# XUANTIE-RV/csi-nn2

Measured on AMD Instinct MI355X. Metric: mobilenetv1_int8_images_per_sec, higher is better.
Workload: dtype i8; 1 GPU; mobilenetv1 int8 NHWC batch 1/GPU, 28 conv layers in 15 launches, hipGraph replay via csinn_*; ops_per_image=1137480704, algorithmic_bytes_per_image=8323144, algorithmic_bytes_per_image_survey=14444616, parallelism=replicas x1

## Files before the change

### csi-nn2_amd/csrc/stemdw_fused.hip

```cpp
#include <stdio.h>
#include <stdlib.h>

#include "dw_patch.h"

namespace shl {

struct StemDwArgs {
    ConvArgs st;
    ConvArgs dw;
    int32_t bh, bw;
    int32_t tiles_x, tiles_y;
    int32_t rw, npx;
    uint32_t rw_magic, bw_magic;
};

template <int EPQ, int EPD>
__global__ __launch_bounds__(256) void stemdw_fused_kernel(StemDwArgs f)
{
    extern __shared__ __attribute__((aligned(16))) char smem[];
    const ConvArgs &q = f.st;
    const ConvArgs &d = f.dw;
    asm volatile("" ::"s"(q.in), "s"(q.w), "s"(q.acc_init), "s"(q.mult), "s"(q.bias), "s"(q.H), "s"(q.W), "s"(q.Ho), "s"(q.Wo), "s"(q.sh),
                 "s"(q.sw), "s"(q.pt), "s"(q.pl), "s"(q.dh), "s"(q.dw), "s"(q.in_zp));
    asm volatile("" ::"s"(f.bh), "s"(f.bw), "s"(f.tiles_y), "s"(f.rw), "s"(f.npx), "s"(f.rw_magic), "s"(f.bw_magic), "s"(d.N), "s"(d.sh),
                 "s"(d.sw), "s"(d.pt), "s"(d.pl), "s"(d.w), "s"(d.acc_init), "s"(d.mult), "s"(d.bias), "s"(d.out));
    asm volatile("" ::"s"(q.out_zp), "s"(q.out_zp_f), "s"(q.clamp_lo), "s"(q.clamp_hi), "s"(d.out_zp), "s"(d.out_zp_f), "s"(d.clamp_lo),
                 "s"(d.clamp_hi), "s"(d.in_zp), "s"(d.Ho), "s"(d.Wo), "s"(d.H), "s"(d.W), "s"(d.C));
    const int tid = threadIdx.x;
    int32_t *w_lds = reinterpret_cast<int32_t *>(smem);
    int32_t *t_tab = w_lds + 7 * 32;
    uint32_t *patch = reinterpret_cast<uint32_t *>(t_tab + 96);
    if (tid < 224) w_lds[tid] = static_cast<const int32_t *>(q.w)[tid];
    if (tid < 96) {
        const int which = tid >> 5, i = tid & 31;
        t_tab[tid] = which == 0 ? q.acc_init[i] : which == 1 ? __float_as_int(q.mult[i]) : __float_as_int(q.bias[i]);
    }
    const int tx = blockIdx.x;
    int ty = blockIdx.y, n = 0;
    if (d.N > 1) {
        n = ty / f.tiles_y;
        ty -= n * f.tiles_y;
    }
    const int oy0 = ty * f.bh, ox0 = tx * f.bw;
    const int ry0 = oy0 * d.sh - d.pt, rx0 = ox0 * d.sw - d.pl;
    const DwThreadConsts dwk = dw_load_consts(d, 0, tid);

    const int8_t *img = static_cast<const int8_t *>(q.in) + (int64_t)n * q.H * q.W * 3;
    const int ntasks = 2 * f.npx;
    const int ppitch = dw_patch_pitch(f.npx);
    const uint32_t zpad = dw_patch_pad(d);
    for (int base = 0; base < ntasks; base += 256) {
        const bool valid = base + tid < ntasks;
        const int task = valid ? base + tid : ntasks - 1;
        const int j = task >> 1, cb = (task & 1) * 16;
        const int pr = (int)(((uint32_t)j * f.rw_magic) >> 20);
        const int pc = j - pr * f.rw;
        const int sy = ry0 + pr, sx = rx0 + pc;
        const bool inside = (unsigned)sy < (unsigned)q.Ho && (unsigned)sx < (unsigned)q.Wo;
        const int y0 = sy * q.sh - q.pt, x0 = sx * q.sw - q.pl;
        int qv[28];
#pragma unroll
        for (int ky = 0; ky < 3; ++ky)
#pragma unroll
            for (int kx = 0; kx < 3; ++kx) {
                const int y = y0 + ky * q.dh, x = x0 + kx * q.dw;
                const bool ok = inside && (unsigned)y < (unsigned)q.H && (unsigned)x < (unsigned)q.W;
                const int8_t *px = img + ((int64_t)y * q.W + x) * 3;
#pragma unroll
                for (int c = 0; c < 3; ++c) qv[(ky * 3 + kx) * 3 + c] = ok ? (int)px[c] : q.in_zp;
            }
        qv[27] = 0;
        uint32_t q4[7];
#pragma unroll
        for (int g = 0; g < 7; ++g)
            q4[g] = (uint32_t)(qv[4 * g] & 0xFF) | ((uint32_t)(qv[4 * g + 1] & 0xFF) << 8) |
                    ((uint32_t)(qv[4 * g + 2] & 0xFF) << 16) | ((uint32_t)(qv[4 * g + 3] & 0xFF) << 24);
        if (base == 0) __syncthreads();
        int acc[16];
#pragma unroll
        for (int e = 0; e < 16; ++e) acc[e] = 0;
#pragma unroll
        for (int g = 0; g < 7; ++g)
#pragma unroll
            for (int v = 0; v < 4; ++v) {
                const int4 w = *reinterpret_cast<const int4 *>(&w_lds[g * 32 + cb + 4 * v]);
                acc[4 * v + 0] = __builtin_amdgcn_sdot4((int)q4[g], w.x, acc[4 * v + 0], false);
                acc[4 * v + 1] = __builtin_amdgcn_sdot4((int)q4[g], w.y, acc[4 * v + 1], false);
                acc[4 * v + 2] = __builtin_amdgcn_sdot4((int)q4[g], w.z, acc[4 * v + 2], false);
                acc[4 * v + 3] = __builtin_amdgcn_sdot4((int)q4[g], w.w, acc[4 * v + 3], false);
            }
#pragma unroll
        for (int v = 0; v < 4; ++v) {
            const int c = cb + 4 * v;
            const int4 ai = *reinterpret_cast<const int4 *>(t_tab + c);
            const float4 mu = *reinterpret_cast<const float4 *>(t_tab + 32 + c);
            const float4 bi = *reinterpret_cast<const float4 *>(t_tab + 64 + c);
            const uint32_t pk = requant4_i8_sel<EPQ>(acc[4 * v] + ai.x, acc[4 * v + 1] + ai.y, acc[4 * v + 2] + ai.z,
                                               acc[4 * v + 3] + ai.w, mu, bi, q);
            if (valid) patch[dw_patch_slot(j, c >> 2, ppitch)] = inside ? pk : zpad;
        }
    }
    __syncthreads();

    DwPatchGeom g;
    g.bh = f.bh, g.bw = f.bw, g.rw = f.rw, g.bw_magic = f.bw_magic, g.pitch = ppitch;
    g.oy0 = oy0, g.ox0 = ox0, g.ry0 = ry0, g.rx0 = rx0, g.n = n, g.ch0 = 0;
    depthwise_from_patch<EPD>(d, patch, g, dwk, tid, 256);
}

static bool stemdw_geometry(const ConvArgs &q, const ConvArgs &d, StemDwArgs &f)
{
    if (q.Kh != 3 || q.Kw != 3 || q.C != 3 || q.Co != 32) return false;
    if (d.Kh != 3 || d.Kw != 3 || d.dh != 1 || d.dw != 1 || d.C != 32 || d.Co != 32) return false;
    if (d.H != q.Ho || d.W != q.Wo || d.N != q.N || d.sh < 1 || d.sh > 2 || d.sw < 1 || d.sw > 2) return false;
    if (d.pt < 0 || d.pl < 0 || d.pt > 2 || d.pl > 2) return false;
    if ((int64_t)d.Ho * d.Wo * d.C >= ((int64_t)1 << 31)) return false;
    f.bh = d.Ho < 2 ? d.Ho : 2;
    f.bw = d.Wo < 28 ? d.Wo : 28;
    if (const char *e = getenv("SHL_MI355X_STEMDW_TILE")) {
        int h = 0, w = 0;
        if (sscanf(e, "%dx%d", &h, &w) == 2 && h > 0 && w > 0) f.bh = h < d.Ho ? h : d.Ho, f.bw = w < d.Wo ? w : d.Wo;
    }
    f.tiles_y = (d.Ho + f.bh - 1) / f.bh;
    f.tiles_x = (d.Wo + f.bw - 1) / f.bw;
    f.rw = (f.bw - 1) * d.sw + 3;
    f.npx = ((f.bh - 1) * d.sh + 3) * f.rw;
    f.rw_magic = ((1u << 20) + f.rw - 1) / f.rw;
    f.bw_magic = ((1u << 20) + f.bw - 1) / f.bw;
    if (f.npx >= 2048 || f.tiles_x > 65535 || (int64_t)f.tiles_y * d.N > 65535) return false;
    return (int64_t)f.tiles_x * f.tiles_y * d.N <= 2048;
}

bool stemdw_fusable(const ConvArgs &q, const ConvArgs &d)
{
    StemDwArgs f;
    return stemdw_geometry(q, d, f);
}

int launch_stemdw_fused(const ConvArgs &q, const ConvArgs &d, hipStream_t s)
{
    StemDwArgs f;
    f.st = q;
    f.dw = d;
    if (!stemdw_geometry(q, d, f)) {
        set_error("stemdw_fused: the pair does not qualify");
        return SHL_MI355X_ENOTSUP;
    }
    const dim3 grid((unsigned)f.tiles_x, (unsigned)(f.tiles_y * d.N));
    const size_t lds = (size_t)(7 * 32 + 96) * 4 + dw_patch_bytes(f.npx);
    const int epq = (q.act != SHL_MI355X_ACT_NONE && !q.act_clamp) ? -1 : (q.div_exact ? 3 : 0);
    const int epd = (d.act != SHL_MI355X_ACT_NONE && !d.act_clamp) ? -1 : (d.div_exact ? 3 : 0);
    if (epq == 3 && epd == 3) hipLaunchKernelGGL((stemdw_fused_kernel<3, 3>), grid, dim3(256), lds, s, f);
    else if (epq == 0 && epd == 0) hipLaunchKernelGGL((stemdw_fused_kernel<0, 0>), grid, dim3(256), lds, s, f);
    else hipLaunchKernelGGL((stemdw_fused_kernel<-1, -1>), grid, dim3(256), lds, s, f);
    SHL_HIP(hipGetLastError());
    return SHL_MI355X_OK;
}

}
```

Baseline: 17580 img/s.

## Compute stem conv with MFMA i8 from an LDS-staged input patch in stem+dw fusion

The stem 3x3x3->32 conv inside the fused stem+depthwise kernel switches from per-thread sdot4 loops (27 global byte loads per task) to a path that first stages the raw input patch into LDS with buffer byte loads. It then builds im2col fragments with alignbyte and runs one mfma_i32_32x32x32_i8 per 32-pixel tile per wave. Weights and requant constants now sit in registers instead of LDS. This is meant to cut redundant global input loads and ALU dot-product work, at the cost of more register pressure, extra LDS for the input patch, and a new launch variant chosen by patch size. It is on by default and can be disabled with an environment variable.

```diff
diff --git a/csi-nn2_amd/csrc/stemdw_fused.hip b/csi-nn2_amd/csrc/stemdw_fused.hip
--- a/csi-nn2_amd/csrc/stemdw_fused.hip
+++ b/csi-nn2_amd/csrc/stemdw_fused.hip
@@ -12,9 +12,13 @@
     int32_t tiles_x, tiles_y;
     int32_t rw, npx;
     uint32_t rw_magic, bw_magic;
+    int32_t mfma;
+    int32_t ir, ipd;
+    uint32_t ipd_magic;
+    int32_t mt;
 };
 
-template <int EPQ, int EPD>
+template <int EPQ, int EPD, bool MFMA, int NI = 0>
 __global__ __launch_bounds__(256) void stemdw_fused_kernel(StemDwArgs f)
 {
     extern __shared__ __attribute__((aligned(16))) char smem[];
@@ -26,15 +30,8 @@
                  "s"(d.sw), "s"(d.pt), "s"(d.pl), "s"(d.w), "s"(d.acc_init), "s"(d.mult), "s"(d.bias), "s"(d.out));
     asm volatile("" ::"s"(q.out_zp), "s"(q.out_zp_f), "s"(q.clamp_lo), "s"(q.clamp_hi), "s"(d.out_zp), "s"(d.out_zp_f), "s"(d.clamp_lo),
                  "s"(d.clamp_hi), "s"(d.in_zp), "s"(d.Ho), "s"(d.Wo), "s"(d.H), "s"(d.W), "s"(d.C));
+    if constexpr (MFMA) asm volatile("" ::"s"(f.ir), "s"(f.ipd), "s"(f.ipd_magic), "s"(f.mt));
     const int tid = threadIdx.x;
-    int32_t *w_lds = reinterpret_cast<int32_t *>(smem);
-    int32_t *t_tab = w_lds + 7 * 32;
-    uint32_t *patch = reinterpret_cast<uint32_t *>(t_tab + 96);
-    if (tid < 224) w_lds[tid] = static_cast<const int32_t *>(q.w)[tid];
-    if (tid < 96) {
-        const int which = tid >> 5, i = tid & 31;
-        t_tab[tid] = which == 0 ? q.acc_init[i] : which == 1 ? __float_as_int(q.mult[i]) : __float_as_int(q.bias[i]);
-    }
     const int tx = blockIdx.x;
     int ty = blockIdx.y, n = 0;
     if (d.N > 1) {
@@ -43,61 +40,158 @@
     }
     const int oy0 = ty * f.bh, ox0 = tx * f.bw;
     const int ry0 = oy0 * d.sh - d.pt, rx0 = ox0 * d.sw - d.pl;
-    const DwThreadConsts dwk = dw_load_consts(d, 0, tid);
-
     const int8_t *img = static_cast<const int8_t *>(q.in) + (int64_t)n * q.H * q.W * 3;
-    const int ntasks = 2 * f.npx;
     const int ppitch = dw_patch_pitch(f.npx);
     const uint32_t zpad = dw_patch_pad(d);
-    for (int base = 0; base < ntasks; base += 256) {
-        const bool valid = base + tid < ntasks;
-        const int task = valid ? base + tid : ntasks - 1;
-        const int j = task >> 1, cb = (task & 1) * 16;
-        const int pr = (int)(((uint32_t)j * f.rw_magic) >> 20);
-        const int pc = j - pr * f.rw;
-        const int sy = ry0 + pr, sx = rx0 + pc;
-        const bool inside = (unsigned)sy < (unsigned)q.Ho && (unsigned)sx < (unsigned)q.Wo;
-        const int y0 = sy * q.sh - q.pt, x0 = sx * q.sw - q.pl;
-        int qv[28];
-#pragma unroll
-        for (int ky = 0; ky < 3; ++ky)
-#pragma unroll
-            for (int kx = 0; kx < 3; ++kx) {
-                const int y = y0 + ky * q.dh, x = x0 + kx * q.dw;
-                const bool ok = inside && (unsigned)y < (unsigned)q.H && (unsigned)x < (unsigned)q.W;
-                const int8_t *px = img + ((int64_t)y * q.W + x) * 3;
-#pragma unroll
-                for (int c = 0; c < 3; ++c) qv[(ky * 3 + kx) * 3 + c] = ok ? (int)px[c] : q.in_zp;
-            }
-        qv[27] = 0;
-        uint32_t q4[7];
-#pragma unroll
-        for (int g = 0; g < 7; ++g)
-            q4[g] = (uint32_t)(qv[4 * g] & 0xFF) | ((uint32_t)(qv[4 * g + 1] & 0xFF) << 8) |
-                    ((uint32_t)(qv[4 * g + 2] & 0xFF) << 16) | ((uint32_t)(qv[4 * g + 3] & 0xFF) << 24);
-        if (base == 0) __syncthreads();
-        int acc[16];
-#pragma unroll
-        for (int e = 0; e < 16; ++e) acc[e] = 0;
-#pragma unroll
-        for (int g = 0; g < 7; ++g)
+    uint32_t *patch;
+    DwThreadConsts dwk;
+
+    if constexpr (MFMA) {
+        const int lane = tid & 63, frow = lane & 31, khalf = lane >> 5;
+        const int wave = __builtin_amdgcn_readfirstlane(tid >> 6);
+        uint32_t *ipatch = reinterpret_cast<uint32_t *>(smem);
+        patch = ipatch + ((f.ir * f.ipd + 3) & ~3);
+        const int iy0 = ry0 * q.sh - q.pt, ib0 = (rx0 * q.sw - q.pl) * 3, rowb = q.W * 3;
+        const __amdgpu_buffer_rsrc_t rsrc = __builtin_amdgcn_make_buffer_rsrc(const_cast<int8_t *>(img), 0, q.H * rowb, 0x00020000);
+        const int nd = f.ir * f.ipd;
+        uint32_t ib[NI][4];
+        bool iok[NI][4];
+#pragma unroll
+        for (int u = 0; u < NI; ++u) {
+            const int i = tid + 256 * u;
+            const int r = (int)(((uint32_t)i * f.ipd_magic) >> 20);
+            const int b = ib0 + 4 * (i - r * f.ipd);
+            const int y = iy0 + r;
+            const bool yok = (unsigned)y < (unsigned)q.H;
+            const int off = y * rowb + b;
+#pragma unroll
+            for (int e = 0; e < 4; ++e) {
+                ib[u][e] = __builtin_amdgcn_raw_buffer_load_b8(rsrc, off + e, 0, 0);
+                iok[u][e] = yok && (unsigned)(b + e) < (unsigned)rowb;
+            }
+        }
+        v4i fa;
+        const int32_t *w = static_cast<const int32_t *>(q.w);
+#pragma unroll
+        for (int j = 0; j < 4; ++j) {
+            const int g = 4 * khalf + j;
+            const int32_t v = w[(g < 7 ? g : 6) * 32 + frow];
+            fa[j] = g < 7 ? v : 0;
+        }
+        float4 mu[4], bi[4];
+        v16i ainit;
+#pragma unroll
+        for (int g = 0; g < 4; ++g) {
+            const int c = 8 * g + 4 * khalf;
+            const int4 ai = *reinterpret_cast<const int4 *>(q.acc_init + c);
+            mu[g] = *reinterpret_cast<const float4 *>(q.mult + c);
+            bi[g] = *reinterpret_cast<const float4 *>(q.bias + c);
+            ainit[4 * g] = ai.x, ainit[4 * g + 1] = ai.y, ainit[4 * g + 2] = ai.z, ainit[4 * g + 3] = ai.w;
+        }
+        dwk = dw_load_consts(d, 0, tid);
+        const uint32_t zb = (uint32_t)(q.in_zp & 0xff);
+#pragma unroll
+        for (int u = 0; u < NI; ++u) {
+            uint32_t v = 0;
+#pragma unroll
+            for (int e = 0; e < 4; ++e) v |= (iok[u][e] ? ib[u][e] : zb) << (8 * e);
+            if (tid + 256 * u < nd) ipatch[tid + 256 * u] = v;
+        }
+        __syncthreads();
+        const int rstep = q.sh * f.ipd * 4, cstep = q.sw * 3;
+        for (int tile = wave; tile < f.mt; tile += 4) {
+            const int jl = tile * 32 + frow;
+            const int j = jl < f.npx ? jl : f.npx - 1;
+            const int pr = (int)(((uint32_t)j * f.rw_magic) >> 20);
+            const int pc = j - pr * f.rw;
+            const bool inside = (unsigned)(ry0 + pr) < (unsigned)q.Ho && (unsigned)(rx0 + pc) < (unsigned)q.Wo;
+            const int o = pr * rstep + pc * cstep;
+            const uint32_t *p = ipatch + (o >> 2);
+            const uint32_t sb = (uint32_t)o & 3;
+            uint32_t r[3][3];
+#pragma unroll
+            for (int ky = 0; ky < 3; ++ky) {
+                const uint32_t v0 = p[ky * f.ipd], v1 = p[ky * f.ipd + 1], v2 = p[ky * f.ipd + 2];
+                r[ky][0] = __builtin_amdgcn_alignbyte(v1, v0, sb);
+                r[ky][1] = __builtin_amdgcn_alignbyte(v2, v1, sb);
+                r[ky][2] = v2 >> (8 * sb);
+            }
+            const uint32_t kd0 = r[0][0], kd1 = r[0][1];
+            const uint32_t kd2 = (r[0][2] & 0xFFu) | (r[1][0] << 8);
+            const uint32_t kd3 = __builtin_amdgcn_alignbyte(r[1][1], r[1][0], 3);
+            const uint32_t kd4 = (r[1][1] >> 24) | ((r[1][2] & 0xFFu) << 8) | (r[2][0] << 16);
+            const uint32_t kd5 = __builtin_amdgcn_alignbyte(r[2][1], r[2][0], 2);
+            const uint32_t kd6 = (r[2][1] >> 16) | ((r[2][2] & 0xFFu) << 16);
+            const bool hi = khalf != 0;
+            const v4i fb = {(int)(hi ? kd4 : kd0), (int)(hi ? kd5 : kd1), (int)(hi ? kd6 : kd2), hi ? 0 : (int)kd3};
+            const v16i acc = __builtin_amdgcn_mfma_i32_32x32x32_i8(fa, fb, ainit, 0, 0, 0);
+#pragma unroll
+            for (int g = 0; g < 4; ++g) {
+                const uint32_t pk = requant4_i8_sel<EPQ>(acc[4 * g], acc[4 * g + 1], acc[4 * g + 2], acc[4 * g + 3], mu[g], bi[g], q);
+                if (jl < f.npx) patch[dw_patch_slot(j, 2 * g + khalf, ppitch)] = inside ? pk : zpad;
+            }
+        }
+    } else {
+        int32_t *w_lds = reinterpret_cast<int32_t *>(smem);
+        int32_t *t_tab = w_lds + 7 * 32;
+        patch = reinterpret_cast<uint32_t *>(t_tab + 96);
+        if (tid < 224) w_lds[tid] = static_cast<const int32_t *>(q.w)[tid];
+        if (tid < 96) {
+            const int which = tid >> 5, i = tid & 31;
+            t_tab[tid] = which == 0 ? q.acc_init[i] : which == 1 ? __float_as_int(q.mult[i]) : __float_as_int(q.bias[i]);
+        }
+        dwk = dw_load_consts(d, 0, tid);
+        const int ntasks = 2 * f.npx;
+        for (int base = 0; base < ntasks; base += 256) {
+            const bool valid = base + tid < ntasks;
+            const int task = valid ? base + tid : ntasks - 1;
+            const int j = task >> 1, cb = (task & 1) * 16;
+            const int pr = (int)(((uint32_t)j * f.rw_magic) >> 20);
+            const int pc = j - pr * f.rw;
+            const int sy = ry0 + pr, sx = rx0 + pc;
+            const bool inside = (unsigned)sy < (unsigned)q.Ho && (unsigned)sx < (unsigned)q.Wo;
+            const int y0 = sy * q.sh - q.pt, x0 = sx * q.sw - q.pl;
+            int qv[28];
+#pragma unroll
+            for (int ky = 0; ky < 3; ++ky)
+#pragma unroll
+                for (int kx = 0; kx < 3; ++kx) {
+                    const int y = y0 + ky * q.dh, x = x0 + kx * q.dw;
+                    const bool ok = inside && (unsigned)y < (unsigned)q.H && (unsigned)x < (unsigned)q.W;
+                    const int8_t *px = img + ((int64_t)y * q.W + x) * 3;
+#pragma unroll
+                    for (int c = 0; c < 3; ++c) qv[(ky * 3 + kx) * 3 + c] = ok ? (int)px[c] : q.in_zp;
+                }
+            qv[27] = 0;
+            uint32_t q4[7];
+#pragma unroll
+            for (int g = 0; g < 7; ++g)
+                q4[g] = (uint32_t)(qv[4 * g] & 0xFF) | ((uint32_t)(qv[4 * g + 1] & 0xFF) << 8) |
+                        ((uint32_t)(qv[4 * g + 2] & 0xFF) << 16) | ((uint32_t)(qv[4 * g + 3] & 0xFF) << 24);
+            if (base == 0) __syncthreads();
+            int acc[16];
+#pragma unroll
+            for (int e = 0; e < 16; ++e) acc[e] = 0;
+#pragma unroll
+            for (int g = 0; g < 7; ++g)
+#pragma unroll
+                for (int v = 0; v < 4; ++v) {
+                    const int4 w = *reinterpret_cast<const int4 *>(&w_lds[g * 32 + cb + 4 * v]);
+                    acc[4 * v + 0] = __builtin_amdgcn_sdot4((int)q4[g], w.x, acc[4 * v + 0], false);
+                    acc[4 * v + 1] = __builtin_amdgcn_sdot4((int)q4[g], w.y, acc[4 * v + 1], false);
+                    acc[4 * v + 2] = __builtin_amdgcn_sdot4((int)q4[g], w.z, acc[4 * v + 2], false);
+                    acc[4 * v + 3] = __builtin_amdgcn_sdot4((int)q4[g], w.w, acc[4 * v + 3], false);
+                }
 #pragma unroll
             for (int v = 0; v < 4; ++v) {
-                const int4 w = *reinterpret_cast<const int4 *>(&w_lds[g * 32 + cb + 4 * v]);
-                acc[4 * v + 0] = __builtin_amdgcn_sdot4((int)q4[g], w.x, acc[4 * v + 0], false);
-                acc[4 * v + 1] = __builtin_amdgcn_sdot4((int)q4[g], w.y, acc[4 * v + 1], false);
-                acc[4 * v + 2] = __builtin_amdgcn_sdot4((int)q4[g], w.z, acc[4 * v + 2], false);
-                acc[4 * v + 3] = __builtin_amdgcn_sdot4((int)q4[g], w.w, acc[4 * v + 3], false);
-            }
-#pragma unroll
-        for (int v = 0; v < 4; ++v) {
-            const int c = cb + 4 * v;
-            const int4 ai = *reinterpret_cast<const int4 *>(t_tab + c);
-            const float4 mu = *reinterpret_cast<const float4 *>(t_tab + 32 + c);
-            const float4 bi = *reinterpret_cast<const float4 *>(t_tab + 64 + c);
-            const uint32_t pk = requant4_i8_sel<EPQ>(acc[4 * v] + ai.x, acc[4 * v + 1] + ai.y, acc[4 * v + 2] + ai.z,
-                                               acc[4 * v + 3] + ai.w, mu, bi, q);
-            if (valid) patch[dw_patch_slot(j, c >> 2, ppitch)] = inside ? pk : zpad;
+                const int c = cb + 4 * v;
+                const int4 ai = *reinterpret_cast<const int4 *>(t_tab + c);
+                const float4 mu = *reinterpret_cast<const float4 *>(t_tab + 32 + c);
+                const float4 bi = *reinterpret_cast<const float4 *>(t_tab + 64 + c);
+                const uint32_t pk = requant4_i8_sel<EPQ>(acc[4 * v] + ai.x, acc[4 * v + 1] + ai.y, acc[4 * v + 2] + ai.z,
+                                                   acc[4 * v + 3] + ai.w, mu, bi, q);
+                if (valid) patch[dw_patch_slot(j, c >> 2, ppitch)] = inside ? pk : zpad;
+            }
         }
     }
     __syncthreads();
@@ -106,6 +200,11 @@
     g.bh = f.bh, g.bw = f.bw, g.rw = f.rw, g.bw_magic = f.bw_magic, g.pitch = ppitch;
     g.oy0 = oy0, g.ox0 = ox0, g.ry0 = ry0, g.rx0 = rx0, g.n = n, g.ch0 = 0;
     depthwise_from_patch<EPD>(d, patch, g, dwk, tid, 256);
+}
+
+static size_t stemdw_lds_bytes(const StemDwArgs &f, bool mfma)
+{
+    return (mfma ? (size_t)((f.ir * f.ipd + 3) & ~3) * 4 : (size_t)(7 * 32 + 96) * 4) + dw_patch_bytes(f.npx);
 }
 
 static bool stemdw_geometry(const ConvArgs &q, const ConvArgs &d, StemDwArgs &f)
@@ -128,6 +227,14 @@
     f.rw_magic = ((1u << 20) + f.rw - 1) / f.rw;
     f.bw_magic = ((1u << 20) + f.bw - 1) / f.bw;
     if (f.npx >= 2048 || f.tiles_x > 65535 || (int64_t)f.tiles_y * d.N > 65535) return false;
+    static const char *mf = getenv("SHL_MI355X_STEMDW_MFMA");
+    f.ir = ((f.bh - 1) * d.sh + 2) * q.sh + 3;
+    const int ic = (f.rw - 1) * q.sw + 3;
+    f.ipd = (3 * ic + 3 + 3) / 4;
+    f.ipd_magic = ((1u << 20) + f.ipd - 1) / f.ipd;
+    f.mt = (f.npx + 31) / 32;
+    f.mfma = !(mf && mf[0] == '0') && q.dh == 1 && q.dw == 1 && (int64_t)q.H * q.W * 3 < ((int64_t)1 << 31) &&
+             f.ir * f.ipd <= 1024 && (int64_t)f.ir * f.ipd * f.ipd < (1 << 20) && stemdw_lds_bytes(f, true) <= 64 * 1024;
     return (int64_t)f.tiles_x * f.tiles_y * d.N <= 2048;
 }
 
@@ -147,12 +254,19 @@
         return SHL_MI355X_ENOTSUP;
     }
     const dim3 grid((unsigned)f.tiles_x, (unsigned)(f.tiles_y * d.N));
-    const size_t lds = (size_t)(7 * 32 + 96) * 4 + dw_patch_bytes(f.npx);
+    const size_t lds = stemdw_lds_bytes(f, f.mfma);
     const int epq = (q.act != SHL_MI355X_ACT_NONE && !q.act_clamp) ? -1 : (q.div_exact ? 3 : 0);
     const int epd = (d.act != SHL_MI355X_ACT_NONE && !d.act_clamp) ? -1 : (d.div_exact ? 3 : 0);
-    if (epq == 3 && epd == 3) hipLaunchKernelGGL((stemdw_fused_kernel<3, 3>), grid, dim3(256), lds, s, f);
-    else if (epq == 0 && epd == 0) hipLaunchKernelGGL((stemdw_fused_kernel<0, 0>), grid, dim3(256), lds, s, f);
-    else hipLaunchKernelGGL((stemdw_fused_kernel<-1, -1>), grid, dim3(256), lds, s, f);
+#define SHL_STEMDW(M, NI)                                                                                        \
+    do {                                                                                                         \
+        if (epq == 3 && epd == 3) hipLaunchKernelGGL((stemdw_fused_kernel<3, 3, M, NI>), grid, dim3(256), lds, s, f);      \
+        else if (epq == 0 && epd == 0) hipLaunchKernelGGL((stemdw_fused_kernel<0, 0, M, NI>), grid, dim3(256), lds, s, f); \
+        else hipLaunchKernelGGL((stemdw_fused_kernel<-1, -1, M, NI>), grid, dim3(256), lds, s, f);                         \
+    } while (0)
+    if (!f.mfma) SHL_STEMDW(false, 0);
+    else if (f.ir * f.ipd <= 512) SHL_STEMDW(true, 2);
+    else SHL_STEMDW(true, 4);
+#undef SHL_STEMDW
     SHL_HIP(hipGetLastError());
     return SHL_MI355X_OK;
 }
```

Measured after the change: 17500 img/s, median of 4. Within noise of the previous version (-0.4%).
